# EIDOSLAB/ProgressiveCodec

Hardware: AMD Instinct MI355X
Metric: megapixels/s encode+decode (256x256 batches) (higher is better)
Workload: dtype f32

## Files before the change

### include/pcodec.h

```cpp
#ifndef PCODEC_H
#define PCODEC_H

#include <stddef.h>
#include <stdint.h>

#ifdef __cplusplus
extern "C" {
#endif

#if defined(__GNUC__)
#define PC_API __attribute__((visibility("default")))
#else
#define PC_API
#endif

enum {
    PC_OK = 0,
    PC_ERR_ARG = -1,
    PC_ERR_INDEX = -2,
    PC_ERR_BUFFER = -3,
    PC_ERR_TRUNCATED = -4,
    PC_ERR_CDF = -5,
    PC_ERR_HIP = -6,
    PC_ERR_NOMEM = -7,
// ... 167 lines not shown
    const float* g1_seg0; const float* g1_w; const float* g1_bias; float* g1_out;
    int tile_cfg;
} pc_test_conv_desc;
#define PC_PLAN_UNI_16_3 1
#define PC_PLAN_UNI_32_2 2
#define PC_PLAN_UNI_32_3 3
#define PC_PLAN_UNI_32_2_SQ 4
#define PC_PLAN_UNI_OTHER 5
#define PC_PLAN_L0_64x64 6
#define PC_PLAN_L0_64x64_SMALLC 7
#define PC_PLAN_L0_128x32 8
#define PC_PLAN_L0_128x32_SMALLC 9
#define PC_PLAN_L0_128x128 10
#define PC_PLAN_L0_128x128_SMALLC 11
#define PC_PLAN_IN_GDN 12
#define PC_FORM_SLOW 1
#define PC_FORM_DIRECT 2
#define PC_FORM_TABLE 3
#define PC_FORM_NCHW_PS 4
#define PC_FORM_L0_DIRECT 5
#define PC_FORM_L0_GENERIC 6
#define PC_FORM_IN_GDN 7
PC_API int pc_test_conv(const pc_test_conv_desc* d, int* plan, void* stream);

typedef struct pc_test_stage_desc {
    int size;
    int kind;
    int B;
    int HW;
    int C;
    int H;
    int W;
    const float* scale;
    int ld_scale;
    const float* mu;
    int ld_mu;
    const float* y;
    int ld_y;
    const float* ybase;
    int ld_ybase;
    const float* yadd;
    int ld_yadd;
    const float* thr;
    int mask_mode;
    const float* mask_src;
    int64_t mask_sb;
// ... 55 lines not shown
```

### progressivecodec_amd/_lib.py

```python
import ctypes as C
import os

_HERE = os.path.dirname(os.path.abspath(__file__))
LIB_PATH = os.environ.get("PC_LIB") or os.path.join(_HERE, "libpcodec.so")

PC_OK = 0
ERRORS = {-1: "PC_ERR_ARG", -2: "PC_ERR_INDEX", -3: "PC_ERR_BUFFER", -4: "PC_ERR_TRUNCATED", -5: "PC_ERR_CDF",
          -6: "PC_ERR_HIP", -7: "PC_ERR_NOMEM", -8: "PC_ERR_STATE", -9: "PC_ERR_MISSING"}

EXPORTS = [
    "pc_version", "pc_strerror", "pc_last_hip_error", "pc_rans_bound", "pc_rans_encode_with_indexes",
    "pc_rans_decode_with_indexes", "pc_rans_encode_batch", "pc_rans_decode_batch", "pc_pmf_to_quantized_cdf",
    "pc_pack_conv_weight", "pc_conv2d_nhwc", "pc_gdn_nhwc", "pc_win_attention_nhwc", "pc_mask_quantile_threshold",
    "pc_gc_prep_encode", "pc_gc_prep_decode_index", "pc_gc_dequantize", "pc_codec_create", "pc_codec_destroy",
    "pc_codec_set_tensor", "pc_codec_set_tables", "pc_codec_finalize", "pc_codec_set_threads", "pc_codec_compress",
    "pc_codec_num_slices", "pc_codec_get_string", "pc_codec_decompress", "pc_codec_read_tap", "pc_codec_read_tap_i32",
    "pc_codec_profile_begin", "pc_codec_profile_end", "pc_codec_compress_levels", "pc_codec_get_level_string",
    "pc_codec_decompress_levels", "pc_codec_forward", "pc_codec_set_cust_map", "pc_codec_strings_size", "pc_codec_copy_strings",
    "pc_codec_decompress_packed", "pc_host_pool_plan", "pc_rans_decode_stream", "pc_codec_set_scale_table", "pc_codec_profile_bytes", "pc_contract_id", "pc_rans_decode_batch_u8", "pc_codec_set_rem",
    "pc_codec_host_stats", "pc_codec_set_rem_checkpoint", "pc_codec_set_option", "pc_selftest_packed_gelu", "pc_profile_set_epoch", "pc_codec_profile_intervals",
    "pc_codec_set_post_filter", "pc_codec_post_filter",
    "pc_codec_set_model", "pc_codec_wacnn_compress", "pc_codec_wacnn_decompress", "pc_codec_wacnn_forward",
    "pc_test_conv", "pc_codec_set_topology", "pc_test_stage",
]


class PcodecError(RuntimeError):
    def __init__(self, code, where=""):
        self.code = code
        msg = lib().pc_strerror(code).decode() if _lib is not None else ""
        hip = lib().pc_last_hip_error() if (_lib is not None and code == -6) else 0
        super().__init__(f"{where}: {ERRORS.get(code, code)} ({msg})" + (f" hipError={hip}" if hip else ""))


_lib = None


def lib():
    global _lib
    if _lib is None:
        if not os.path.exists(LIB_PATH):
            raise ImportError(
                f"{LIB_PATH} not found: build it with `python -c 'import __graft_entry__ as g; g.build()'` "
                "(hipcc --offload-arch=gfx950).  progressivecodec_amd has no CPU fallback.")
        L = C.CDLL(LIB_PATH)
        vp, i32p, f32p, u8p, sz = C.c_void_p, C.POINTER(C.c_int32), C.POINTER(C.c_float), C.POINTER(C.c_uint8), C.c_size_t
# ... 13 lines not shown
        L.pc_pmf_to_quantized_cdf.argtypes = [vp, C.c_int, C.c_int, vp]
        L.pc_pack_conv_weight.argtypes = [vp, C.c_int, C.c_int, C.c_int, C.c_int, vp]
        L.pc_conv2d_nhwc.argtypes = [vp, C.c_int, C.c_int, C.c_int, C.c_int, vp, vp, C.c_int, C.c_int, C.c_int, C.c_int,
                                     C.c_int, C.c_int, vp, vp]
        L.pc_gdn_nhwc.argtypes = [vp, C.c_int, C.c_int, C.c_int, C.c_int, vp, vp, C.c_int, vp, vp]
        L.pc_win_attention_nhwc.argtypes = [vp, vp, C.c_int, C.c_int, C.c_int, C.c_int, C.c_int, C.c_int, C.c_int, vp, vp]
        L.pc_mask_quantile_threshold.argtypes = [vp, C.c_int, C.c_int, C.c_int, C.c_int, C.c_float, vp, vp]
        L.pc_gc_prep_encode.argtypes = [vp, C.c_int, vp, C.c_int, vp, C.c_int, vp, C.c_int, vp, C.c_int, C.c_int, C.c_int,
                                        vp, C.c_int, C.c_float, vp, vp, vp, vp, C.c_int, vp]
        L.pc_gc_prep_decode_index.argtypes = [vp, C.c_int, vp, C.c_int, C.c_int, C.c_int, vp, C.c_int, C.c_float, vp, vp, vp]
        L.pc_gc_dequantize.argtypes = [vp, vp, C.c_int, C.c_int, C.c_int, vp, C.c_int, vp]
        L.pc_codec_create.argtypes = [C.POINTER(vp), C.c_int]
        L.pc_codec_destroy.argtypes = [vp]
        L.pc_codec_destroy.restype = None
        L.pc_codec_set_tensor.argtypes = [vp, C.c_char_p, vp, C.c_int, C.POINTER(C.c_int64), C.c_int]
        L.pc_codec_set_tables.argtypes = [vp, C.c_int, vp, C.c_int, C.c_int, vp, vp]
        L.pc_codec_finalize.argtypes = [vp]
        L.pc_codec_set_threads.argtypes = [vp, C.c_int]
        L.pc_codec_set_option.argtypes = [vp, C.c_char_p, C.c_int]
        if hasattr(L, "pc_selftest_packed_gelu"):
            L.pc_selftest_packed_gelu.argtypes = [C.POINTER(C.c_uint64), C.POINTER(C.c_uint64)]
        if hasattr(L, "pc_test_conv"):
            L.pc_test_conv.argtypes = [vp, C.POINTER(C.c_int), vp]
        if hasattr(L, "pc_test_stage"):
            L.pc_test_stage.argtypes = [vp, C.POINTER(C.c_int), vp]
        L.pc_codec_compress.argtypes = [vp, vp, C.c_int, C.c_int, C.c_int, C.c_double, C.c_int, vp, vp]
        L.pc_codec_num_slices.argtypes = [vp]
        L.pc_codec_get_string.argtypes = [vp, C.c_int, C.c_int, C.POINTER(vp), C.POINTER(sz)]
        L.pc_codec_decompress.argtypes = [vp, vp, vp, C.c_int, vp, vp, C.c_int, C.c_int, C.c_int, C.c_double, C.c_int, vp, vp]
        L.pc_codec_compress_levels.argtypes = [vp, vp, C.c_int, C.c_int, C.c_int, vp, C.c_int, C.c_int, vp, vp]
        L.pc_codec_get_level_string.argtypes = [vp, C.c_int, C.c_int, C.c_int, C.POINTER(vp), C.POINTER(sz)]
        L.pc_codec_decompress_levels.argtypes = [vp, vp, vp, vp, vp, C.c_int, C.c_int, C.c_int, vp, C.c_int, C.c_int, vp, vp]
        L.pc_codec_set_cust_map.argtypes = [vp, vp]
        L.pc_codec_set_rem.argtypes = [vp, vp, C.c_int]
        L.pc_codec_set_rem_checkpoint.argtypes = [vp, vp]
        L.pc_codec_set_post_filter.argtypes = [vp, C.c_int]
        L.pc_codec_post_filter.argtypes = [vp, C.c_int, vp, C.c_int, C.c_int, C.c_int, vp, vp]
        L.pc_codec_set_model.argtypes = [vp, C.c_int]
        L.pc_codec_set_topology.argtypes = [vp, vp]
        L.pc_codec_wacnn_compress.argtypes = [vp, vp, C.c_int, C.c_int, C.c_int, vp]
        L.pc_codec_wacnn_decompress.argtypes = [vp, vp, sz, vp, vp, C.c_int, C.c_int, C.c_int, vp, vp]
        L.pc_codec_wacnn_forward.argtypes = [vp, vp, C.c_int, C.c_int, C.c_int, vp, vp, vp, vp]
        L.pc_codec_strings_size.argtypes = [vp, C.POINTER(sz), C.POINTER(C.c_int)]
        L.pc_codec_copy_strings.argtypes = [vp, vp, sz, vp, sz]
        L.pc_codec_decompress_packed.argtypes = [vp, vp, vp, C.c_int, C.c_int, C.c_int, vp, C.c_int, C.c_int, vp, vp]
        L.pc_codec_forward.argtypes = [vp, vp, C.c_int, C.c_int, C.c_int, C.c_double, C.c_int, vp, vp, vp, vp, C.c_int, vp]
# ... 17 lines not shown
```

### progressivecodec_amd/csrc/pc_codec.hip

```cpp
#include <hip/hip_runtime.h>

#include <algorithm>
#include <atomic>
#include <chrono>
#include <condition_variable>
#include <new>
#include <cmath>
#include <cstdio>
#include <cstdlib>
#include <cstring>
#include <functional>
#include <map>
#include <mutex>
#include <thread>
#include <string>
#include <vector>

#include "../../include/pcodec.h"
#include "pc_device.h"
#include "pc_host.h"

static std::atomic<int> g_last_hip{0};
struct pc_codec;
static thread_local pc_codec* g_prof = nullptr;
// ... 45 lines not shown
    pc_rowtab_cache* rowtabs = nullptr;
    std::map<std::string, HostTensor> sd;
    std::vector<void*> weight_allocs;
    std::map<std::string, DevBuf> bufs;
    struct GaW { ConvW c0, c2, c5, c7; GdnW g1, g3, g6; WamW w4, w8; };
    GaW ga[2];
    std::vector<LrrW> rem;
    int rem_levels_loaded = 0;
    int rem_n = 0;
    double rem_check[3] = {0, 0, 0};
    bool multi_enc = false;
    GsW gs[2];
    int post_mode = 0;
    UnetW unet[2];
    ConvW ha[5];
    HsW hms[2], hss[2];
    pc_topology topo{};
    ConvW joiner[NS0][3];
    Stack5W cc_mean[NS0], cc_scale[NS0], lrp[NS0], cc_mean_p[NS0], cc_scale_p[NS0], lrp_p[NS0];
    float* medians = nullptr;
    const float* cust_map = nullptr;
    const float* rem_ckpt = nullptr;
    int opt_serial = 0, opt_lanes_enc = 0, opt_lanes_dec = 0;
    int rem_mu_std = 0;
    float* eb_net = nullptr;
    float* scale_table = nullptr;
    int n_table = 0;
    float scale_bound = 0.11f;
    Tables gc, eb;
    int32_t* h_sym = nullptr; int32_t* h_idx = nullptr; size_t h_cap = 0;
    int res_slices = 0, res_B = 0;
    std::vector<char> res_level_coded;
    std::vector<hipEvent_t> lvl_events;
    hipStream_t pipe_stream = nullptr;
    std::vector<hipEvent_t> pipe_ev;
    std::vector<std::vector<uint8_t>> y_strings;
    std::vector<std::vector<uint8_t>> z_strings;
    int n_threads = 0;
    bool profile = false;
    bool profile_in_schedule = false;
    bool serial_profile() const { return profile && !profile_in_schedule; }
    std::mutex prof_mu;
    std::vector<hipEvent_t> ev;
    size_t ev_used = 0;
    double prof_flops = 0.0, prof_bytes = 0.0;
    struct ProfRec { int M, N, K, nphase, epi; double flops, bytes; double t0_ms, t1_ms; };
// ... 32 lines not shown
    ~LaunchState() { g_prof = prof0; g_rowtabs = rowtabs0; }
    LaunchState(const LaunchState&) = delete;
    LaunchState& operator=(const LaunchState&) = delete;
};

double now_ms() { return std::chrono::duration<double, std::milli>(std::chrono::steady_clock::now().time_since_epoch()).count(); }

int launch_conv(const pc_conv_params& q_in, hipStream_t st, int* plan = nullptr)
{
    pc_conv_params q = q_in;
    q.rowtab_cache = g_rowtabs;
    pc_codec* c = g_prof;
    if (!c) return pc_conv_launch(q, st, plan);
    long taps = 0;
    for (int ph = 0; ph < q.nphase; ++ph) taps += q.ntap[ph];
    const double ng = q.ngroup == 2 ? 2.0 : 1.0;
    double fl = 2.0 * (double)q.M * (double)q.Cout * (double)taps * (double)q.Cin * ng;
    if (q.fg_gamma) fl += 2.0 * (double)q.M * (double)q.Cout * (double)q.Cout;
    double by = 0.0;
    for (int sg = 0; sg < q.nseg; ++sg) by += 4.0 * (double)q.B * q.H * q.W * q.seg[sg].nch * (sg == 0 ? ng : 1.0);
    by += ng * 4.0 * ((double)taps * q.Cin * q.Cout + q.Cout);
    if (q.fg_gamma) by += 4.0 * ((double)q.Cout * q.Cout + q.Cout);
    by += ng * 4.0 * (double)q.nphase * q.M * q.Cout;
    if (q.aux0 && q.epi != PC_EPI_NONE && q.epi != PC_EPI_GELU && q.epi != PC_EPI_CLAMP01) by += 4.0 * (double)q.nphase * q.M * q.Cout;
    if (q.aux1 && (q.epi == PC_EPI_GATE || q.epi == PC_EPI_LRP_ADD)) by += 4.0 * (double)q.nphase * q.M * q.Cout;
    hipEvent_t e0, e1;
    {
        std::lock_guard<std::mutex> lk(c->prof_mu);
        if (c->ev_used + 2 > c->ev.size()) {
            const size_t old = c->ev.size();
            c->ev.resize(old + 512);
            for (size_t i = old; i < c->ev.size(); ++i) HIPCHK(hipEventCreate(&c->ev[i]));
        }
        c->prof_flops += fl;
        c->prof_bytes += by;
        c->prof_rec.push_back({q.M, q.Cout, (int)(taps * q.Cin / q.nphase), q.nphase, q.epi, fl, by, 0.0, 0.0});
        e0 = c->ev[c->ev_used++]; e1 = c->ev[c->ev_used++];
    }
    HIPCHK(hipEventRecord(e0, st));
    const int r = pc_conv_launch(q, st, plan);
    HIPCHK(hipEventRecord(e1, st));
    return r;
}

const HostTensor* find(const pc_codec* c, const std::string& k, int dtype, std::initializer_list<int64_t> shape)
{
    auto it = c->sd.find(k);
// ... 168 lines not shown
    PCCHK(load_conv(c, n + "up2.0", 64, 128, 1, 0, &u->up2));
    PCCHK(load_cbr(c, n + "up_conv2", 64, 16, &u->u2));
    PCCHK(load_conv(c, p + ".1", 16, 3, 3, 0, &u->out));
    return PC_OK;
}

int load_stack5(pc_codec* c, const std::string& p, int Cin, Stack5W* s)
{
    int ci = Cin;
    for (int j = 0; j < 5; ++j) { PCCHK(load_conv(c, p + "." + std::to_string(2 * j), ci, CC_W[j], 3, 0, &s->c[j])); ci = CC_W[j]; }
    return PC_OK;
}

int load_hs(pc_codec* c, const std::string& p, HsW* h)
{
    PCCHK(load_conv(c, p + ".0", NCH, 192, 3, 0, &h->c0));
    PCCHK(load_conv(c, p + ".2.0", 192, 224 * 4, 3, 0, &h->c2));
    PCCHK(load_conv(c, p + ".4", 224, 256, 3, 0, &h->c4));
    PCCHK(load_conv(c, p + ".6.0", 256, 288 * 4, 3, 0, &h->c6));
    PCCHK(load_conv(c, p + ".8", 288, D0, 3, 0, &h->c8));
    return PC_OK;
}

struct Seg { const float* p; int ld; int nch; };

void fill_conv_taps(pc_conv_params& q, int k, int stride)
{
    const int pad = k / 2;
    q.nphase = 1; q.ntap[0] = k * k; q.stride = stride;
    for (int ky = 0; ky < k; ++ky)
        for (int kx = 0; kx < k; ++kx) {
            const int t = ky * k + kx;
            q.dy[0][t] = (ky - pad); q.dx[0][t] = (kx - pad); q.wtap[0][t] = t;
        }
    q.osy = q.osx = 1; q.ooy[0] = q.oox[0] = 0;
}

void fill_subpixel_taps(pc_conv_params& q)
{
    q.nphase = 1; q.ntap[0] = 9; q.stride = 1; q.osy = q.osx = 1; q.ooy[0] = q.oox[0] = 0;
    for (int t = 0; t < 9; ++t) { q.dy[0][t] = 1 - t / 3; q.dx[0][t] = 1 - t % 3; q.wtap[0][t] = t; }
}

void fill_deconv_taps(pc_conv_params& q)
{
    q.nphase = 4; q.stride = 1; q.osy = q.osx = 2;
// ... 11 lines not shown
        }
}

int conv_geometry(pc_conv_params& q, int kind, int k, int stride, int H, int W, int B, bool pixel_shuffle)
{
    if (B <= 0 || H <= 0 || W <= 0) return PC_ERR_ARG;
    q.B = B; q.H = H; q.W = W;
    q.Ho = H; q.Wo = W;
    if (kind == 0) {
        if (k <= 0 || k > 5 || stride <= 0) return PC_ERR_ARG;
        fill_conv_taps(q, k, stride);
        q.Ho = (H + 2 * (k / 2) - k) / stride + 1;
        q.Wo = (W + 2 * (k / 2) - k) / stride + 1;
    } else if (kind == 1) fill_deconv_taps(q);
    else if (kind == 2) fill_subpixel_taps(q);
    else return PC_ERR_ARG;
    q.outH = q.osy * q.Ho; q.outW = q.osx * q.Wo;
    q.M = B * q.Ho * q.Wo;
    q.pixel_shuffle = (pixel_shuffle || kind == 2) ? 1 : 0;
    if (q.pixel_shuffle) { q.outH *= 2; q.outW *= 2; }
    return PC_OK;
}

struct Group1 { const ConvW* w; const float* seg0; float* out; };

int conv_n(hipStream_t st, const ConvW& w, const Seg* segs, int nseg, int B, int H, int W, int stride,
           float* out, int ldo, int epi, const float* aux0 = nullptr, int ld0 = 0, const float* aux1 = nullptr, int ld1 = 0,
           bool pixel_shuffle = false, const Group1* g1 = nullptr, float* out_relu = nullptr)
{
    pc_conv_params q;
    std::memset(&q, 0, sizeof(q));
    int cin = 0;
    for (int j = 0; j < nseg; ++j) {
        const Seg& s = segs[j];
        if (s.nch == 0) continue;
        if (q.nseg >= PC_MAX_SEG) return PC_ERR_ARG;
        q.seg[q.nseg].ptr = s.p; q.seg[q.nseg].ld = s.ld; q.seg[q.nseg].nch = s.nch; ++q.nseg; cin += s.nch;
    }
    if (cin != w.Cin) return PC_ERR_ARG;
    q.Cin = cin;
    q.w = w.w; q.wlayout = w.layout; q.bias = w.b; q.Cout = w.Cout;
    q.epi = epi; q.aux0 = aux0; q.ld0 = ld0; q.aux1 = aux1; q.ld1 = ld1;
    q.out = out; q.out_relu = out_relu;
    PCCHK(conv_geometry(q, w.kind == 0 ? 0 : 1, w.k, stride, H, W, B, pixel_shuffle));
    q.out_sc = 1; q.out_sx = ldo; q.out_sy = (int64_t)q.outW * ldo; q.out_sb = (int64_t)q.outH * q.outW * ldo;
    if (g1) {
        if (g1->w->Cin != w.Cin || g1->w->Cout != w.Cout || g1->w->k != w.k || g1->w->layout != 1 || w.layout != 1) return PC_ERR_ARG;
        q.ngroup = 2; q.g1_seg0 = g1->seg0; q.g1_w = g1->w->w; q.g1_bias = g1->w->b; q.g1_out = g1->out;
    }
    return launch_conv(q, st);
}

int conv(hipStream_t st, const ConvW& w, std::initializer_list<Seg> segs, int B, int H, int W, int stride,
         float* out, int ldo, int epi, const float* aux0 = nullptr, int ld0 = 0, const float* aux1 = nullptr, int ld1 = 0,
         bool pixel_shuffle = false, const Group1* g1 = nullptr, float* out_relu = nullptr)
{
    return conv_n(st, w, segs.begin(), (int)segs.size(), B, H, W, stride, out, ldo, epi, aux0, ld0, aux1, ld1, pixel_shuffle, g1, out_relu);
}

int gdn(hipStream_t st, const GdnW& g, const float* x, int B, int H, int W, bool inverse, float* out, int* plan = nullptr)
{
    pc_conv_params q;
    std::memset(&q, 0, sizeof(q));
    q.nseg = 1; q.seg[0].ptr = x; q.seg[0].ld = g.C; q.seg[0].nch = g.C; q.Cin = g.C;
    q.B = B; q.H = H; q.W = W; q.square = 1;
    fill_conv_taps(q, 1, 1);
    q.w = g.gamma; q.wlayout = 1; q.bias = g.beta; q.Cout = g.C;
    q.Ho = H; q.Wo = W; q.outH = H; q.outW = W; q.M = B * H * W;
    q.out = out; q.out_sc = 1; q.out_sx = g.C; q.out_sy = (int64_t)W * g.C; q.out_sb = (int64_t)H * W * g.C;
    q.epi = inverse ? PC_EPI_IGDN : PC_EPI_GDN; q.aux0 = x; q.ld0 = g.C;
    return launch_conv(q, st, plan);
}

int ru(hipStream_t st, const RuW& r, const float* x, int C, int B, int H, int W, float* t1, float* t2, float* out)
{
    PCCHK(conv(st, r.c0, {{x, C, C}}, B, H, W, 1, t1, C / 2, PC_EPI_GELU));
    PCCHK(conv(st, r.c2, {{t1, C / 2, C / 2}}, B, H, W, 1, t2, C / 2, PC_EPI_GELU));
    PCCHK(conv(st, r.c4, {{t2, C / 2, C / 2}}, B, H, W, 1, out, C, PC_EPI_RES_GELU, x, C));
    return PC_OK;
}

int wam(pc_codec* c, hipStream_t st, const WamW& w, const float* x, int B, int H, int W, float* out, int ldo = 0)
{
    const int C = w.C;
    if (ldo == 0) ldo = C;
    const size_t M = (size_t)B * H * W;
    float *t1, *t2, *a0, *a1, *qkv, *o;
    PCCHK(c->buf("wam_t1", M * (C / 2), &t1));
    PCCHK(c->buf("wam_t2", M * (C / 2), &t2));
    PCCHK(c->buf("wam_a0", M * C, &a0));
    PCCHK(c->buf("wam_a1", M * C, &a1));
    PCCHK(c->buf("wam_b0", M * C, &o));
    PCCHK(c->buf("wam_qkv", M * 3 * C, &qkv));
    float* b1;
    PCCHK(c->buf("wam_b1", M * C, &b1));
    PCCHK(ru(st, w.a[0], x, C, B, H, W, t1, t2, a0));
    PCCHK(ru(st, w.a[1], a0, C, B, H, W, t1, t2, a1));
    PCCHK(ru(st, w.a[2], a1, C, B, H, W, t1, t2, a0));
    PCCHK(conv(st, w.qkv, {{x, C, C}}, B, H, W, 1, qkv, 3 * C, PC_EPI_NONE));
    PCCHK(pc_win_attention_launch(qkv, w.bias, B, H, W, C, HEADS, w.ws, w.shift, (float)std::pow((double)(C / HEADS), -0.5), a1, st, 1));
    PCCHK(conv(st, w.proj, {{a1, C, C}}, B, H, W, 1, o, C, PC_EPI_RES, x, C));
    PCCHK(ru(st, w.b[0], o, C, B, H, W, t1, t2, b1));
    PCCHK(ru(st, w.b[1], b1, C, B, H, W, t1, t2, o));
    PCCHK(ru(st, w.b[2], o, C, B, H, W, t1, t2, b1));
    PCCHK(conv(st, w.out, {{b1, C, C}}, B, H, W, 1, out, ldo, PC_EPI_GATE, a0, C, x, C));
    return PC_OK;
}

int stack5_n(pc_codec* c, hipStream_t st, const Stack5W& s, const Seg* segs, int nseg, int B, int h, int w, float* out, int ldo, int epi,
             const char* tag, const float* aux0 = nullptr, int ld0 = 0, const float* aux1 = nullptr, int ld1 = 0)
{
    const size_t M = (size_t)B * h * w;
    float *t0, *t1;
    PCCHK(c->buf(std::string(tag) + "_t0", M * 224, &t0));
    PCCHK(c->buf(std::string(tag) + "_t1", M * 176, &t1));
    PCCHK(conv_n(st, s.c[0], segs, nseg, B, h, w, 1, t0, 224, PC_EPI_GELU));
    PCCHK(conv(st, s.c[1], {{t0, 224, 224}}, B, h, w, 1, t1, 176, PC_EPI_GELU));
    PCCHK(conv(st, s.c[2], {{t1, 176, 176}}, B, h, w, 1, t0, 128, PC_EPI_GELU));
// ... 240 lines not shown
    HIPCHK(hipHostMalloc(reinterpret_cast<void**>(&c->h_idx), n_int32 * 4, hipHostMallocDefault));
    c->h_cap = n_int32;
    return PC_OK;
}

int mask_mode_for(int mask_pol, double quality, float* q_out)
{
    if (mask_pol == PC_MASK_TWO_LEVELS) return quality == 0 ? 3 : 2;
    if (mask_pol == PC_MASK_THREE_LEVELS_STD) {
        if (quality == 0) return 3;
        if (quality == 2) return 2;
        *q_out = (float)0.8;
        return 1;
    }
    if (quality >= 10) return 2;
    if (quality == 0) return 3;
    const double pr = quality * 0.1;
    *q_out = (float)(1.0 - pr);
    return 1;
}

int hyper(pc_codec* c, hipStream_t st, const float* z_hat, int B, int zh, int zw, double quality, float* lm, float* ls)
{
    if (quality != 0 && c->topo.single_hyperprior) {
        PCCHK(hs(c, st, c->hss[1], z_hat, B, zh, zw, ls, MLAT));
        PCCHK(hs(c, st, c->hms[1], z_hat, B, zh, zw, lm, MLAT));
        return PC_OK;
    }
    PCCHK(hs(c, st, c->hss[0], z_hat, B, zh, zw, ls, MLAT));
    PCCHK(hs(c, st, c->hms[0], z_hat, B, zh, zw, lm, MLAT));
    if (quality != 0) {
        PCCHK(hs(c, st, c->hss[1], z_hat, B, zh, zw, ls + D0, MLAT));
        PCCHK(hs(c, st, c->hms[1], z_hat, B, zh, zw, lm + D0, MLAT));
    }
    return PC_OK;
}

}

extern "C" int pc_pack_conv_weight(const float* w, int kind, int Cout, int Cin, int k, float* out)
{
    if (!w || !out || Cout <= 0 || Cin <= 0 || k <= 0) return PC_ERR_ARG;
    if (kind == 2) {
        if (Cout != 3 || k != 5 || Cin % 16) return PC_ERR_ARG;
        pack_deconv3_subpixel(w, Cin, out);
        return PC_OK;
// ... 16 lines not shown
                    float* dst = out + (((size_t)(ky * k + kx) * Cout) + co) * Cin;
                    for (int ci = 0; ci < Cin; ++ci) dst[ci] = src(co, ci, ky, kx);
                }
    }
    return PC_OK;
}

extern "C" int pc_conv2d_nhwc(const float* x, int B, int H, int W, int Cin, const float* w_packed, const float* bias,
                              int kind, int Cout, int k, int stride, int act, int tile_cfg, float* out, void* stream)
{
    if (!x || !w_packed || !out) return PC_ERR_ARG;
    pc_conv_params q;
    std::memset(&q, 0, sizeof(q));
    q.nseg = 1; q.seg[0].ptr = x; q.seg[0].ld = Cin; q.seg[0].nch = Cin; q.Cin = Cin;
    if (Cin % 16) { q.smallc = 1; q.in_sc = 1; q.in_sx = Cin; q.in_sy = (int64_t)W * Cin; q.in_sb = (int64_t)H * W * Cin; if (kind != 0) return PC_ERR_ARG; }
    q.w = w_packed; q.bias = bias; q.Cout = Cout; q.epi = act ? PC_EPI_GELU : PC_EPI_NONE; q.tile_cfg = tile_cfg;
    q.wlayout = pc_conv_weight_layout(kind, Cin, Cout, k);
    if (kind != 0 && k != 5) return PC_ERR_ARG;
    PCCHK(conv_geometry(q, kind == 0 ? 0 : 1, k, stride, H, W, B, false));
    q.out = out; q.out_sc = 1; q.out_sx = Cout; q.out_sy = (int64_t)q.outW * Cout; q.out_sb = (int64_t)q.outH * q.outW * Cout;
    return pc_conv_launch(q, (hipStream_t)stream);
}

extern "C" int pc_test_conv(const pc_test_conv_desc* d, int* plan, void* stream)
{
    if (plan) plan[0] = plan[1] = 0;
    if (!d || !d->out || !d->w || d->nseg < 1 || d->nseg > PC_MAX_SEG || d->B <= 0 || d->H <= 0 || d->W <= 0) return PC_ERR_ARG;
    pc_conv_params q;
    std::memset(&q, 0, sizeof(q));
    q.nseg = d->nseg;
    for (int s = 0; s < d->nseg; ++s) { q.seg[s].ptr = d->seg_ptr[s]; q.seg[s].ld = d->seg_ld[s]; q.seg[s].nch = d->seg_nch[s]; }
    q.smallc = d->smallc ? 1 : 0;
    q.in_sb = d->in_sb; q.in_sy = d->in_sy; q.in_sx = d->in_sx; q.in_sc = d->in_sc;
    q.Cin = d->Cin;
    q.square = d->square ? 1 : 0;
    q.w = d->w; q.bias = d->bias; q.Cout = d->Cout; q.tile_cfg = d->tile_cfg;
    q.epi = d->epi; q.aux0 = d->aux0; q.ld0 = d->ld0; q.aux1 = d->aux1; q.ld1 = d->ld1;
    q.fg_gamma = d->fg_gamma; q.fg_beta = d->fg_beta;
    if (d->kind == 2 && d->Cout != 12) return PC_ERR_ARG;
    PCCHK(conv_geometry(q, d->kind, d->k, d->stride, d->H, d->W, d->B, d->pixel_shuffle != 0));
    if (d->kind == 0) q.wlayout = q.square ? 1 : pc_conv_weight_layout(0, d->Cin, d->Cout, d->k);
    else q.wlayout = d->kind == 1 ? pc_conv_weight_layout(1, d->Cin, d->Cout, 5) : 1;
    q.out = d->out; q.out_sb = d->out_sb; q.out_sy = d->out_sy; q.out_sx = d->out_sx; q.out_sc = d->out_sc;
    q.out_relu = d->out_relu;
    if (d->ngroup == 2) { q.ngroup = 2; q.g1_seg0 = d->g1_seg0; q.g1_w = d->g1_w; q.g1_bias = d->g1_bias; q.g1_out = d->g1_out; }
    return pc_conv_launch(q, (hipStream_t)stream, plan);
}

extern "C" int pc_test_stage(const pc_test_stage_desc* d, int* plan, void* stream)
{
    if (plan) plan[0] = 0;
    if (!d || d->size != (int)sizeof(pc_test_stage_desc)) return PC_ERR_ARG;
    hipStream_t st = (hipStream_t)stream;
    int chosen = 0, rc = PC_ERR_ARG;
    switch (d->kind) {
    case PC_STAGE_PREP_ENC: case PC_STAGE_PREP_DEC_INDEX: case PC_STAGE_PREP_DEQUANT: {
        pc_prep_params p;
        std::memset(&p, 0, sizeof(p));
        p.B = d->B; p.HW = d->HW; p.C = d->C;
        p.scale = d->scale; p.ld_scale = d->ld_scale; p.mu = d->mu; p.ld_mu = d->ld_mu; p.y = d->y; p.ld_y = d->ld_y;
        p.ybase = d->ybase; p.ld_ybase = d->ld_ybase; p.yadd = d->yadd; p.ld_yadd = d->ld_yadd;
        p.thr = d->thr; p.mask_mode = d->mask_mode; p.mask_src = d->mask_src; p.mask_sb = d->mask_sb;
        p.table = d->table; p.ntable = d->ntable; p.bound = d->bound;
        p.sym = d->sym; p.idx = d->idx; p.idx8 = d->idx8; p.mask = d->mask; p.yhat = d->yhat; p.ld_yhat = d->ld_yhat;
        p.lik = d->lik; p.lik_sb = d->lik_sb;
        if (d->kind == PC_STAGE_PREP_ENC) {
            if (!p.scale || !p.mu || !p.y || !p.sym || !p.idx || !p.yhat || !p.table || (p.mask_mode == 1 && !p.thr)) return PC_ERR_ARG;
            rc = pc_prep_enc_launch(p, st, &chosen);
// ... 165 lines not shown
        for (int j = 0; j + 1 < sizes[i]; ++j) if (row[j + 1] <= row[j]) return PC_ERR_CDF;
    }
    Tables& t = which == 0 ? c->gc : c->eb;
    t.cdf.assign(cdf, cdf + (size_t)n_cdf * cdf_stride);
    t.len.assign(sizes, sizes + n_cdf);
    t.off.assign(offsets, offsets + n_cdf);
    t.n = n_cdf; t.stride = cdf_stride;
    t.lut.assign((size_t)n_cdf * 256, 0);
    pc::build_decode_lut(t.cdf.data(), t.n, t.stride, t.len.data(), t.lut.data());
    return PC_OK;
}

extern "C" int pc_codec_set_threads(pc_codec* c, int n) { if (!c) return PC_ERR_ARG; c->n_threads = n; return PC_OK; }

extern "C" int pc_codec_set_option(pc_codec* c, const char* name, int value)
{
    if (!c || !name || value < 0) return PC_ERR_ARG;
    const std::string n(name);
    if (n == "serial_schedule") c->opt_serial = value ? 1 : 0;
    else if (n == "lanes_enc") { if (value > 8) return PC_ERR_ARG; c->opt_lanes_enc = value; }
    else if (n == "lanes_dec") { if (value > 8) return PC_ERR_ARG; c->opt_lanes_dec = value; }
    else if (n == "host_threads") c->n_threads = value;
    else if (n == "profile_in_schedule") c->profile_in_schedule = value != 0;
    else return PC_ERR_ARG;
    return PC_OK;
}

namespace {

int load_ga(pc_codec* c, const std::string& p, int Cy, pc_codec::GaW* g)
{
    PCCHK(load_conv(c, p + ".0", 3, NCH, 5, 0, &g->c0));
    PCCHK(load_gdn(c, p + ".1", NCH, &g->g1));
    PCCHK(load_conv(c, p + ".2", NCH, NCH, 5, 0, &g->c2));
    PCCHK(load_gdn(c, p + ".3", NCH, &g->g3));
    PCCHK(load_wam(c, p + ".4", NCH, 8, 4, &g->w4));
    PCCHK(load_conv(c, p + ".5", NCH, NCH, 5, 0, &g->c5));
    PCCHK(load_gdn(c, p + ".6", NCH, &g->g6));
    PCCHK(load_conv(c, p + ".7", NCH, Cy, 5, 0, &g->c7));
    return load_wam(c, p + ".8", Cy, 4, 2, &g->w8);
}

int load_gs(pc_codec* c, const std::string& p, GsW* g)
{
    PCCHK(load_wam(c, p + ".0", D0, 4, 2, &g->w0));
    PCCHK(load_conv(c, p + ".1", D0, NCH, 5, 1, &g->d1));
// ... 30 lines not shown
    if (!c->multi_enc) PCCHK(load_ga(c, "g_a", MLAT, &c->ga[0]));
    else for (int k = 0; k < 2; ++k) PCCHK(load_ga(c, "g_a." + std::to_string(k), D0, &c->ga[k]));
    for (int k = 0; k < 2; ++k) PCCHK(load_gs(c, "g_s." + std::to_string(k), &c->gs[k]));
    PCCHK(load_ha(c, MLAT));
    if (c->topo.single_hyperprior) {
        for (int which = 0; which < 2; ++which) {
            const std::string p = which == 0 ? "h_mean_s" : "h_scale_s";
            HsW* h = which == 0 ? c->hms : c->hss;
            PCCHK(load_conv(c, p + ".0", NCH, 192, 3, 0, &h[1].c0));
            PCCHK(load_conv(c, p + ".2.0", 192, 224 * 4, 3, 0, &h[1].c2));
            PCCHK(load_conv(c, p + ".4", 224, 256, 3, 0, &h[1].c4));
            PCCHK(load_conv(c, p + ".6.0", 256, 288 * 4, 3, 0, &h[1].c6));
            PCCHK(load_conv(c, p + ".8", 288, MLAT, 3, 0, &h[1].c8));
            const HostTensor* w = find(c, p + ".8.weight", PC_F32, {MLAT, 288, 3, 3});
            const HostTensor* b = find(c, p + ".8.bias", PC_F32, {MLAT});
            if (!w || !b) return PC_ERR_MISSING;
            HostTensor lw{std::vector<uint8_t>(w->data.begin(), w->data.begin() + (size_t)D0 * 288 * 9 * 4), {D0, 288, 3, 3}, PC_F32};
            HostTensor lb{std::vector<uint8_t>(b->data.begin(), b->data.begin() + (size_t)D0 * 4), {D0}, PC_F32};
            c->sd[p + ".8lo.weight"] = std::move(lw);
            c->sd[p + ".8lo.bias"] = std::move(lb);
            h[0] = h[1];
            PCCHK(load_conv(c, p + ".8lo", 288, D0, 3, 0, &h[0].c8));
        }
    } else {
        for (int k = 0; k < 2; ++k) {
            PCCHK(load_hs(c, "h_mean_s." + std::to_string(k), &c->hms[k]));
            PCCHK(load_hs(c, "h_scale_s." + std::to_string(k), &c->hss[k]));
        }
    }
    const int S = 5 - c->topo.support_deficit;
    PCCHK(load_base_stacks(c));
    for (int i = 0; i < NS0; ++i) {
        const std::string s = "." + std::to_string(i);
        PCCHK(load_stack5(c, "cc_mean_transforms_prog" + s, D0 + 32 * std::min(i + 1, S + 1), &c->cc_mean_p[i]));
        PCCHK(load_stack5(c, "cc_scale_transforms_prog" + s, D0 + 32 * std::min(i + 1, S + 1), &c->cc_scale_p[i]));
        PCCHK(load_stack5(c, "lrp_transforms_prog" + s, D0 + 32 * std::min(i + 2, S + 2), &c->lrp_p[i]));
        if (c->topo.joiner_cond) {
            PCCHK(load_conv(c, "joiner" + s + ".0", 2 * SLICE, 64, 3, 0, &c->joiner[i][0]));
            PCCHK(load_conv(c, "joiner" + s + ".2", 64, 64, 3, 0, &c->joiner[i][1]));
            PCCHK(load_conv(c, "joiner" + s + ".4", 64, SLICE, 3, 0, &c->joiner[i][2]));
        }
    }
    return PC_OK;
}

int load_wacnn(pc_codec* c)
{
    c->multi_enc = false;
    PCCHK(load_ga(c, "g_a", D0, &c->ga[0]));
    PCCHK(load_gs(c, "g_s", &c->gs[0]));
    PCCHK(load_ha(c, D0));
    PCCHK(load_hs(c, "h_mean_s", &c->hms[0]));
    PCCHK(load_hs(c, "h_scale_s", &c->hss[0]));
    return load_base_stacks(c);
}

}

extern "C" int pc_codec_finalize(pc_codec* c)
{
    if (!c) return PC_ERR_ARG;
    if (c->finalized) return PC_OK;
    HIPCHK(hipSetDevice(c->device));
    PCCHK(c->model == PC_MODEL_WACNN ? load_wacnn(c) : load_channel(c));
    {
        const HostTensor* q = find(c, "entropy_bottleneck.quantiles", PC_F32, {NCH, 1, 3});
        if (!q) return PC_ERR_MISSING;
        std::vector<float> med(NCH);
        for (int i = 0; i < NCH; ++i) med[i] = reinterpret_cast<const float*>(q->data.data())[3 * i + 1];
        PCCHK(upload(c, med, &c->medians));
    }
    {
        static const int F[6] = {1, 3, 3, 3, 3, 1};
        std::vector<float> net((size_t)NCH * PC_EB_NET_FLOATS, 0.0f);
        bool ok = true;
        for (int i = 0; i < 5 && ok; ++i) {
// ... 1315 lines not shown
```

### progressivecodec_amd/csrc/pc_conv.hip

```cpp
#include <hip/hip_runtime.h>
#include <stdint.h>
#include <algorithm>
#include <atomic>
#include <cstdio>
#include <cstdlib>
#include <cstring>
#include <mutex>
#include <new>
#include <type_traits>
#include <unordered_map>
#include <utility>
#include <vector>

#include "../../include/pc_math.h"
#include "pc_device.h"

typedef float f32x16 __attribute__((ext_vector_type(16)));
typedef float f32x4 __attribute__((ext_vector_type(4)));

namespace {

__device__ __forceinline__ float epilogue_apply(int epi, float v, float a0, float a1)
{
    switch (epi) {
// ... 883 lines not shown
    if (nlive == TN) kloop(std::integral_constant<int, TN>{});
    else if (nlive == 0) kloop(std::integral_constant<int, 0>{});
    else kloop(std::integral_constant<int, 1>{});
    if (DBG & 64) tl[2] = __builtin_amdgcn_s_memrealtime();
    __builtin_amdgcn_s_barrier();
    auto stamp_out = [&]() {
        if (!(DBG & 64) || lane != 0 || blockIdx.x >= 8192 / 4) return;
        asm volatile("s_waitcnt vmcnt(0)" ::: "memory");
        unsigned long long* d = pc_dbg_stamps[blockIdx.x * 4 + wave];
        d[0] = tl[0]; d[1] = tl[1]; d[2] = tl[2]; d[3] = __builtin_amdgcn_s_memrealtime();
        d[4] = (unsigned long long)__builtin_amdgcn_s_getreg(0xF804);
        d[5] = (unsigned long long)__builtin_amdgcn_s_getreg(0xF814);
        d[6] = (unsigned long long)nlive; d[7] = (unsigned long long)blockIdx.x;
    };

    if (nlive == 0) { stamp_out(); return; }
    const bool u0 = epilogue_uses_aux0(p.epi), u1 = epilogue_uses_aux1(p.epi);
    const uint32_t epi_bytes = !p.dense_out ? 0u : (u1 ? 32768u : (u0 ? 16384u : 0u));
    const uint32_t tab_byte0 = (uint32_t)(S * STAGE * 16) > epi_bytes ? (uint32_t)(S * STAGE * 16) : epi_bytes;
    uint32_t* rowtab_lds = reinterpret_cast<uint32_t*>(reinterpret_cast<char*>(smem) + tab_byte0) + wave * 64;
    const uint32_t rowtab_lds_addr = smem_lds + tab_byte0 + (uint32_t)wave * 256u;
    const bool fast = TM * TN == 1 && p.out_sc == 1 && (p.dense_out || !u0) && p.epi != PC_EPI_SE_ADD;
    const int ooy_ph = p.ooy[phase], oox_ph = p.oox[phase];
    const float* const aux0_p = p.aux0; const float* const aux1_p = p.aux1;
    const int ld0_v = p.ld0, ld1_v = p.ld1, epi_v = p.epi;
    const int e_Cout = p.Cout, e_M = p.M, e_dense = p.dense_out, e_perm = p.rowperm, e_ps = p.pixel_shuffle, e_osy = p.osy, e_osx = p.osx, e_Wo = p.Wo,
              e_outH = p.outH, e_outW = p.outW;
    const int64_t e_sx = p.out_sx, e_sy = p.out_sy, e_sb = p.out_sb, e_sc = p.out_sc;
    const int* const e_rowtab = p.rowtab;
    float* const e_relu = p.out_relu;
    auto slow_tile = [&](auto i_tag, auto j_tag) __attribute__((always_inline)) {
        constexpr int i = decltype(i_tag)::value, j = decltype(j_tag)::value;
        const int mb = m0 + wm * 32 * TM + i * 32, nb = n0 + (wn * TN + j) * 32;
        const int n = nb + l31;
        const float bv = (bias && n < e_Cout) ? bias[n] : 0.0f;
        for (int r = 0; r < 16; ++r) {
            const int row = (r & 3) + 8 * (r >> 2) + 4 * half;
            const int m = mb + row;
            if (m >= e_M || n >= e_Cout) continue;
            int64_t opix;
            float v = acc[i][j][r];
            if (bias) v = v + bv;
            if (e_dense) {
                opix = e_perm ? (int64_t)e_rowtab[m] : (int64_t)m;
                const float a1 = epi_v == PC_EPI_SE_ADD ? aux1_p[(opix / HoWo) * ld1_v + n] : (u1 ? aux1_p[opix * ld1_v + n] : 0.0f);
                v = epilogue_apply(epi_v, v, u0 ? aux0_p[opix * ld0_v + n] : 0.0f, a1);
                outp[opix * e_sx + (int64_t)n * e_sc] = v;
// ... 632 lines not shown
```

### progressivecodec_amd/csrc/pc_device.h

```cpp
#ifndef PC_DEVICE_H
#define PC_DEVICE_H

#include <hip/hip_runtime.h>
#include <stdint.h>

#include "../../include/pcodec.h"

#ifdef PC_TUNING
#include <cstdlib>
static inline long pc_tune(const char* name, long dflt) { const char* v = std::getenv(name); return v ? std::atol(v) : dflt; }
#else
static inline constexpr long pc_tune(const char*, long dflt) { return dflt; }
#endif

#define PC_MAX_SEG 8
#define PC_MAX_TAP 25

enum {
    PC_EPI_NONE = 0,
    PC_EPI_GELU = 1,
    PC_EPI_RES_GELU = 2,
    PC_EPI_RES = 3,
    PC_EPI_GATE = 4,
    PC_EPI_GDN = 5,
// ... 25 lines not shown
    int nphase;
    int ntap[4];
    int dy[4][PC_MAX_TAP], dx[4][PC_MAX_TAP];
    int wtap[4][PC_MAX_TAP];
    int stride;
    const float* w;
    int wlayout;
    const float* bias;
    int Cout;
    int Ho, Wo, M;
    int osy, osx, ooy[4], oox[4];
    int outH, outW;
    int64_t out_sb, out_sy, out_sx, out_sc;
    float* out;
    int pixel_shuffle;
    float* out_relu;
    int epi;
    const float* aux0; int ld0;
    const float* aux1; int ld1;
    int tile_cfg;
    const float* fg_gamma; const float* fg_beta;
    int ngroup;
    const float* g1_seg0; const float* g1_w; const float* g1_bias; float* g1_out;
    const int* rowtab;
    void* rowtab_cache;
    int ident_rows;
    int dense_out;
    int rowperm;
    int group_xcd;
    int dbg;
};

int pc_conv_launch(const pc_conv_params& p, hipStream_t stream, int* plan = nullptr);
struct pc_rowtab_cache;
pc_rowtab_cache* pc_rowtab_cache_create(size_t cap_bytes);
void pc_rowtab_cache_destroy(pc_rowtab_cache* c);
size_t pc_rowtab_cache_bytes(pc_rowtab_cache* c);
int pc_conv_weight_layout(int kind, int Cin, int Cout, int k);

int pc_win_attention_launch(const float* qkv, const float* bias, int B, int H, int W, int C, int heads, int ws,
                            int shift, float scale, float* out, hipStream_t stream, int bias_ji = 0, int* plan = nullptr);

struct pc_prep_params {
    int B, HW, C;
    const float* scale; int ld_scale;
    const float* mu; int ld_mu;
// ... 40 lines not shown
```

Baseline: 47.58.

## Batch sibling convolutions into grouped launches in attention and hyper-synthesis

Independent sibling branches run as paired grouped-conv launches instead of sequential ones. In the window attention module the a- and b-branch residual units go through ru_pair, with a per-group residual aux pointer added to the conv kernel. In hyper-synthesis the first convolution of all scale/mean nets is concatenated into one wide conv, and later layers are grouped pairwise. The goal is better GPU occupancy on small spatial sizes and fewer launches, at the cost of extra scratch buffers and a duplicated first-layer weight copy.

```diff
diff --git a/include/pcodec.h b/include/pcodec.h
--- a/include/pcodec.h
+++ b/include/pcodec.h
@@ -213,6 +213,7 @@
 #define PC_FORM_L0_GENERIC 6
 #define PC_FORM_IN_GDN 7
 PC_API int pc_test_conv(const pc_test_conv_desc* d, int* plan, void* stream);
+PC_API int pc_test_conv_g1aux(const pc_test_conv_desc* d, const float* g1_aux0, int* plan, void* stream);
 
 typedef struct pc_test_stage_desc {
     int size;
diff --git a/progressivecodec_amd/_lib.py b/progressivecodec_amd/_lib.py
--- a/progressivecodec_amd/_lib.py
+++ b/progressivecodec_amd/_lib.py
@@ -21,7 +21,7 @@
     "pc_codec_host_stats", "pc_codec_set_rem_checkpoint", "pc_codec_set_option", "pc_selftest_packed_gelu", "pc_profile_set_epoch", "pc_codec_profile_intervals",
     "pc_codec_set_post_filter", "pc_codec_post_filter",
     "pc_codec_set_model", "pc_codec_wacnn_compress", "pc_codec_wacnn_decompress", "pc_codec_wacnn_forward",
-    "pc_test_conv", "pc_codec_set_topology", "pc_test_stage",
+    "pc_test_conv", "pc_codec_set_topology", "pc_test_stage", "pc_test_conv_g1aux",
 ]
 
 
@@ -81,6 +81,8 @@
             L.pc_selftest_packed_gelu.argtypes = [C.POINTER(C.c_uint64), C.POINTER(C.c_uint64)]
         if hasattr(L, "pc_test_conv"):
             L.pc_test_conv.argtypes = [vp, C.POINTER(C.c_int), vp]
+        if hasattr(L, "pc_test_conv_g1aux"):
+            L.pc_test_conv_g1aux.argtypes = [vp, vp, C.POINTER(C.c_int), vp]
         if hasattr(L, "pc_test_stage"):
             L.pc_test_stage.argtypes = [vp, C.POINTER(C.c_int), vp]
         L.pc_codec_compress.argtypes = [vp, vp, C.c_int, C.c_int, C.c_int, C.c_double, C.c_int, vp, vp]
diff --git a/progressivecodec_amd/csrc/pc_codec.hip b/progressivecodec_amd/csrc/pc_codec.hip
--- a/progressivecodec_amd/csrc/pc_codec.hip
+++ b/progressivecodec_amd/csrc/pc_codec.hip
@@ -91,6 +91,8 @@
     const float* cust_map = nullptr;
     const float* rem_ckpt = nullptr;
     int opt_serial = 0, opt_lanes_enc = 0, opt_lanes_dec = 0;
+    int opt_group_siblings = (int)pc_tune("PC_GROUP_SIBLINGS", 1);
+    ConvW hs_c0_cat2, hs_c0_cat4;
     int rem_mu_std = 0;
     float* eb_net = nullptr;
     float* scale_table = nullptr;
@@ -169,7 +171,7 @@
     by += ng * 4.0 * ((double)taps * q.Cin * q.Cout + q.Cout);
     if (q.fg_gamma) by += 4.0 * ((double)q.Cout * q.Cout + q.Cout);
     by += ng * 4.0 * (double)q.nphase * q.M * q.Cout;
-    if (q.aux0 && q.epi != PC_EPI_NONE && q.epi != PC_EPI_GELU && q.epi != PC_EPI_CLAMP01) by += 4.0 * (double)q.nphase * q.M * q.Cout;
+    if (q.aux0 && q.epi != PC_EPI_NONE && q.epi != PC_EPI_GELU && q.epi != PC_EPI_CLAMP01) by += (q.g1_aux0 ? ng : 1.0) * 4.0 * (double)q.nphase * q.M * q.Cout;
     if (q.aux1 && (q.epi == PC_EPI_GATE || q.epi == PC_EPI_LRP_ADD)) by += 4.0 * (double)q.nphase * q.M * q.Cout;
     hipEvent_t e0, e1;
     {
@@ -384,6 +386,25 @@
     return PC_OK;
 }
 
+int load_hs_cat(pc_codec* c, std::initializer_list<std::string> prefixes, ConvW* out)
+{
+    const int n = (int)prefixes.size();
+    std::vector<float> w, bias;
+    for (const std::string& p : prefixes) {
+        const HostTensor* wt = find(c, p + ".0.weight", PC_F32, {192, NCH, 3, 3});
+        const HostTensor* bt = find(c, p + ".0.bias", PC_F32, {192});
+        if (!wt || !bt) { std::fprintf(stderr, "[pcodec] missing/mis-shaped tensor %s.0\n", p.c_str()); return PC_ERR_MISSING; }
+        w.insert(w.end(), reinterpret_cast<const float*>(wt->data.data()), reinterpret_cast<const float*>(wt->data.data()) + (size_t)192 * NCH * 9);
+        bias.insert(bias.end(), reinterpret_cast<const float*>(bt->data.data()), reinterpret_cast<const float*>(bt->data.data()) + 192);
+    }
+    std::vector<float> packed(w.size());
+    PCCHK(pc_pack_conv_weight(w.data(), 0, n * 192, NCH, 3, packed.data()));
+    PCCHK(upload(c, packed, &out->w));
+    PCCHK(upload(c, bias, &out->b));
+    out->Cin = NCH; out->Cout = n * 192; out->k = 3; out->kind = 0; out->layout = pc_conv_weight_layout(0, NCH, n * 192, 3);
+    return PC_OK;
+}
+
 struct Seg { const float* p; int ld; int nch; };
 
 void fill_conv_taps(pc_conv_params& q, int k, int stride)
@@ -441,7 +462,7 @@
     return PC_OK;
 }
 
-struct Group1 { const ConvW* w; const float* seg0; float* out; };
+struct Group1 { const ConvW* w; const float* seg0; float* out; const float* aux0 = nullptr; };
 
 int conv_n(hipStream_t st, const ConvW& w, const Seg* segs, int nseg, int B, int H, int W, int stride,
            float* out, int ldo, int epi, const float* aux0 = nullptr, int ld0 = 0, const float* aux1 = nullptr, int ld1 = 0,
@@ -465,7 +486,7 @@
     q.out_sc = 1; q.out_sx = ldo; q.out_sy = (int64_t)q.outW * ldo; q.out_sb = (int64_t)q.outH * q.outW * ldo;
     if (g1) {
         if (g1->w->Cin != w.Cin || g1->w->Cout != w.Cout || g1->w->k != w.k || g1->w->layout != 1 || w.layout != 1) return PC_ERR_ARG;
-        q.ngroup = 2; q.g1_seg0 = g1->seg0; q.g1_w = g1->w->w; q.g1_bias = g1->w->b; q.g1_out = g1->out;
+        q.ngroup = 2; q.g1_seg0 = g1->seg0; q.g1_w = g1->w->w; q.g1_bias = g1->w->b; q.g1_out = g1->out; q.g1_aux0 = g1->aux0;
     }
     return launch_conv(q, st);
 }
@@ -496,6 +517,18 @@
     PCCHK(conv(st, r.c0, {{x, C, C}}, B, H, W, 1, t1, C / 2, PC_EPI_GELU));
     PCCHK(conv(st, r.c2, {{t1, C / 2, C / 2}}, B, H, W, 1, t2, C / 2, PC_EPI_GELU));
     PCCHK(conv(st, r.c4, {{t2, C / 2, C / 2}}, B, H, W, 1, out, C, PC_EPI_RES_GELU, x, C));
+    return PC_OK;
+}
+
+int ru_pair(hipStream_t st, const RuW& ra, const RuW& rb, const float* xa, const float* xb, int C, int B, int H, int W,
+            float* ta1, float* ta2, float* tb1, float* tb2, float* outa, float* outb)
+{
+    Group1 g{&rb.c0, xb, tb1};
+    PCCHK(conv(st, ra.c0, {{xa, C, C}}, B, H, W, 1, ta1, C / 2, PC_EPI_GELU, nullptr, 0, nullptr, 0, false, &g));
+    g = Group1{&rb.c2, tb1, tb2};
+    PCCHK(conv(st, ra.c2, {{ta1, C / 2, C / 2}}, B, H, W, 1, ta2, C / 2, PC_EPI_GELU, nullptr, 0, nullptr, 0, false, &g));
+    g = Group1{&rb.c4, tb2, outb, xb};
+    PCCHK(conv(st, ra.c4, {{ta2, C / 2, C / 2}}, B, H, W, 1, outa, C, PC_EPI_RES_GELU, xa, C, nullptr, 0, false, &g));
     return PC_OK;
 }
 
@@ -513,6 +546,19 @@
     PCCHK(c->buf("wam_qkv", M * 3 * C, &qkv));
     float* b1;
     PCCHK(c->buf("wam_b1", M * C, &b1));
+    if (c->opt_group_siblings && (long)((M + 31) / 32) * ((C / 2 + 31) / 32) < 4096 && w.a[0].c0.layout == 1 && w.a[0].c2.layout == 1 && w.a[0].c4.layout == 1) {
+        float *u1, *u2;
+        PCCHK(c->buf("wam_u1", M * (C / 2), &u1));
+        PCCHK(c->buf("wam_u2", M * (C / 2), &u2));
+        PCCHK(conv(st, w.qkv, {{x, C, C}}, B, H, W, 1, qkv, 3 * C, PC_EPI_NONE));
+        PCCHK(pc_win_attention_launch(qkv, w.bias, B, H, W, C, HEADS, w.ws, w.shift, (float)std::pow((double)(C / HEADS), -0.5), a1, st, 1));
+        PCCHK(conv(st, w.proj, {{a1, C, C}}, B, H, W, 1, o, C, PC_EPI_RES, x, C));
+        PCCHK(ru_pair(st, w.a[0], w.b[0], x, o, C, B, H, W, t1, t2, u1, u2, a0, b1));
+        PCCHK(ru_pair(st, w.a[1], w.b[1], a0, b1, C, B, H, W, t1, t2, u1, u2, a1, o));
+        PCCHK(ru_pair(st, w.a[2], w.b[2], a1, o, C, B, H, W, t1, t2, u1, u2, a0, b1));
+        PCCHK(conv(st, w.out, {{b1, C, C}}, B, H, W, 1, out, ldo, PC_EPI_GATE, a0, C, x, C));
+        return PC_OK;
+    }
     PCCHK(ru(st, w.a[0], x, C, B, H, W, t1, t2, a0));
     PCCHK(ru(st, w.a[1], a0, C, B, H, W, t1, t2, a1));
     PCCHK(ru(st, w.a[2], a1, C, B, H, W, t1, t2, a0));
@@ -799,6 +845,37 @@
 
 int hyper(pc_codec* c, hipStream_t st, const float* z_hat, int B, int zh, int zw, double quality, float* lm, float* ls)
 {
+    if (c->opt_group_siblings) {
+        const bool one = quality != 0 && c->topo.single_hyperprior;
+        const int n = (quality != 0 && !one) ? 4 : 2;
+        const HsW* nets[4] = {&c->hss[one ? 1 : 0], &c->hms[one ? 1 : 0], &c->hss[1], &c->hms[1]};
+        float* outs[4] = {ls, lm, ls + D0, lm + D0};
+        const ConvW& cat = n == 4 ? c->hs_c0_cat4 : c->hs_c0_cat2;
+        if (!cat.w || cat.Cout != n * 192 || cat.layout != 1) return PC_ERR_STATE;
+        const size_t M = (size_t)B * zh * zw;
+        float *t0, *t1[4], *t2[4], *t3[4];
+        PCCHK(c->buf("hs_c0", M * 4 * 192, &t0));
+        for (int j = 0; j < n; ++j) {
+            const std::string s = std::to_string(j);
+            PCCHK(c->buf("hs_t1_" + s, M * 4 * 224, &t1[j]));
+            PCCHK(c->buf("hs_t2_" + s, M * 4 * 256, &t2[j]));
+            PCCHK(c->buf("hs_t3_" + s, M * 16 * 288, &t3[j]));
+        }
+        const int ld = n * 192;
+        PCCHK(conv(st, cat, {{z_hat, 192, 192}}, B, zh, zw, 1, t0, ld, PC_EPI_GELU));
+        for (int p = 0; p < n; p += 2) {
+            const HsW &a = *nets[p], &b = *nets[p + 1];
+            Group1 g{&b.c2, t0 + 192 * (p + 1), t1[p + 1]};
+            PCCHK(conv(st, a.c2, {{t0 + 192 * p, ld, 192}}, B, zh, zw, 1, t1[p], 224, PC_EPI_GELU, nullptr, 0, nullptr, 0, true, &g));
+            g = Group1{&b.c4, t1[p + 1], t2[p + 1]};
+            PCCHK(conv(st, a.c4, {{t1[p], 224, 224}}, B, 2 * zh, 2 * zw, 1, t2[p], 256, PC_EPI_GELU, nullptr, 0, nullptr, 0, false, &g));
+            g = Group1{&b.c6, t2[p + 1], t3[p + 1]};
+            PCCHK(conv(st, a.c6, {{t2[p], 256, 256}}, B, 2 * zh, 2 * zw, 1, t3[p], 288, PC_EPI_GELU, nullptr, 0, nullptr, 0, true, &g));
+            g = Group1{&b.c8, t3[p + 1], outs[p + 1]};
+            PCCHK(conv(st, a.c8, {{t3[p], 288, 288}}, B, 4 * zh, 4 * zw, 1, outs[p], MLAT, PC_EPI_NONE, nullptr, 0, nullptr, 0, false, &g));
+        }
+        return PC_OK;
+    }
     if (quality != 0 && c->topo.single_hyperprior) {
         PCCHK(hs(c, st, c->hss[1], z_hat, B, zh, zw, ls, MLAT));
         PCCHK(hs(c, st, c->hms[1], z_hat, B, zh, zw, lm, MLAT));
@@ -861,9 +938,12 @@
     return pc_conv_launch(q, (hipStream_t)stream);
 }
 
-extern "C" int pc_test_conv(const pc_test_conv_desc* d, int* plan, void* stream)
+extern "C" int pc_test_conv(const pc_test_conv_desc* d, int* plan, void* stream) { return pc_test_conv_g1aux(d, nullptr, plan, stream); }
+
+extern "C" int pc_test_conv_g1aux(const pc_test_conv_desc* d, const float* g1_aux0, int* plan, void* stream)
 {
     if (plan) plan[0] = plan[1] = 0;
+    if (g1_aux0 && (!d || d->ngroup != 2)) return PC_ERR_ARG;
     if (!d || !d->out || !d->w || d->nseg < 1 || d->nseg > PC_MAX_SEG || d->B <= 0 || d->H <= 0 || d->W <= 0) return PC_ERR_ARG;
     pc_conv_params q;
     std::memset(&q, 0, sizeof(q));
@@ -882,7 +962,7 @@
     else q.wlayout = d->kind == 1 ? pc_conv_weight_layout(1, d->Cin, d->Cout, 5) : 1;
     q.out = d->out; q.out_sb = d->out_sb; q.out_sy = d->out_sy; q.out_sx = d->out_sx; q.out_sc = d->out_sc;
     q.out_relu = d->out_relu;
-    if (d->ngroup == 2) { q.ngroup = 2; q.g1_seg0 = d->g1_seg0; q.g1_w = d->g1_w; q.g1_bias = d->g1_bias; q.g1_out = d->g1_out; }
+    if (d->ngroup == 2) { q.ngroup = 2; q.g1_seg0 = d->g1_seg0; q.g1_w = d->g1_w; q.g1_bias = d->g1_bias; q.g1_out = d->g1_out; q.g1_aux0 = g1_aux0; }
     return pc_conv_launch(q, (hipStream_t)stream, plan);
 }
 
@@ -1094,6 +1174,7 @@
     else if (n == "lanes_dec") { if (value > 8) return PC_ERR_ARG; c->opt_lanes_dec = value; }
     else if (n == "host_threads") c->n_threads = value;
     else if (n == "profile_in_schedule") c->profile_in_schedule = value != 0;
+    else if (n == "group_siblings") { if (value > 1) return PC_ERR_ARG; c->opt_group_siblings = value; }
     else return PC_ERR_ARG;
     return PC_OK;
 }
@@ -1170,11 +1251,14 @@
             h[0] = h[1];
             PCCHK(load_conv(c, p + ".8lo", 288, D0, 3, 0, &h[0].c8));
         }
+        PCCHK(load_hs_cat(c, {"h_scale_s", "h_mean_s"}, &c->hs_c0_cat2));
     } else {
         for (int k = 0; k < 2; ++k) {
             PCCHK(load_hs(c, "h_mean_s." + std::to_string(k), &c->hms[k]));
             PCCHK(load_hs(c, "h_scale_s." + std::to_string(k), &c->hss[k]));
         }
+        PCCHK(load_hs_cat(c, {"h_scale_s.0", "h_mean_s.0"}, &c->hs_c0_cat2));
+        PCCHK(load_hs_cat(c, {"h_scale_s.0", "h_mean_s.0", "h_scale_s.1", "h_mean_s.1"}, &c->hs_c0_cat4));
     }
     const int S = 5 - c->topo.support_deficit;
     PCCHK(load_base_stacks(c));
@@ -1200,6 +1284,7 @@
     PCCHK(load_ha(c, D0));
     PCCHK(load_hs(c, "h_mean_s", &c->hms[0]));
     PCCHK(load_hs(c, "h_scale_s", &c->hss[0]));
+    PCCHK(load_hs_cat(c, {"h_scale_s", "h_mean_s"}, &c->hs_c0_cat2));
     return load_base_stacks(c);
 }
 
diff --git a/progressivecodec_amd/csrc/pc_conv.hip b/progressivecodec_amd/csrc/pc_conv.hip
--- a/progressivecodec_amd/csrc/pc_conv.hip
+++ b/progressivecodec_amd/csrc/pc_conv.hip
@@ -929,7 +929,8 @@
     const uint32_t rowtab_lds_addr = smem_lds + tab_byte0 + (uint32_t)wave * 256u;
     const bool fast = TM * TN == 1 && p.out_sc == 1 && (p.dense_out || !u0) && p.epi != PC_EPI_SE_ADD;
     const int ooy_ph = p.ooy[phase], oox_ph = p.oox[phase];
-    const float* const aux0_p = p.aux0; const float* const aux1_p = p.aux1;
+    const float* const aux0_p = (p.ngroup == 2 && zsel == 1 && p.g1_aux0) ? p.g1_aux0 : p.aux0;
+    const float* const aux1_p = p.aux1;
     const int ld0_v = p.ld0, ld1_v = p.ld1, epi_v = p.epi;
     const int e_Cout = p.Cout, e_M = p.M, e_dense = p.dense_out, e_perm = p.rowperm, e_ps = p.pixel_shuffle, e_osy = p.osy, e_osx = p.osx, e_Wo = p.Wo,
               e_outH = p.outH, e_outW = p.outW;
diff --git a/progressivecodec_amd/csrc/pc_device.h b/progressivecodec_amd/csrc/pc_device.h
--- a/progressivecodec_amd/csrc/pc_device.h
+++ b/progressivecodec_amd/csrc/pc_device.h
@@ -71,6 +71,7 @@
     const float* fg_gamma; const float* fg_beta;
     int ngroup;
     const float* g1_seg0; const float* g1_w; const float* g1_bias; float* g1_out;
+    const float* g1_aux0;
     const int* rowtab;
     void* rowtab_cache;
     int ident_rows;
```

After: 48.45 (median of 6 runs). +1.8%, better.
